# timsainb/noisereduce

Hardware: AMD Instinct MI355X
Metric: Msamples/s reduce_noise (48 kHz mono, n_fft=1024) (higher is better)
Workload: dtype f32

## Files before the change

noisereduce_amd/csrc/onepass.hpp:

```cpp
#pragma once
#include "fastpath.hpp"

namespace sg {
namespace fast {

constexpr int OP_XW = 9;
constexpr int OP_TILE_WORDS = 16 * OP_XW * 2;
constexpr int OP_MAX_NT = 16;
constexpr int OP_KP = 528;
constexpr int OP_TAB_WIN = 0, OP_TAB_WSQ = 4096, OP_TAB_INVN = 8192, OP_TAB_TW512 = 9216, OP_TAB_TW1024 = 13312,
              OP_TAB_WIN64 = 17408, OP_TAB_TW64 = 25600, OP_TAB_MCONST = 33792, OP_TAB_EXP8 = 35328, OP_TAB_BYTES = 37376;

#ifndef OP_LATE_ARGS
#define OP_LATE_ARGS 1
#endif
#ifndef OP_TRACE
#define OP_TRACE 0
#endif
#ifndef OP_ARGCHECK
#define OP_ARGCHECK 0
#endif
#ifndef OP_TILECOUNT
#define OP_TILECOUNT 0
#endif
// ... 25 lines not shown
#ifndef OP_RESTAGE
#define OP_RESTAGE 0
#endif
#ifndef OP_MAX_ITERS
#define OP_MAX_ITERS 0
#endif
#ifndef OP_LATE_START_US
#define OP_LATE_START_US 0
#endif
#ifndef OP_EXP_STALL_NS
#define OP_EXP_STALL_NS 0
#endif
#ifndef OP_INPLACE
#define OP_INPLACE 0
#endif
struct OnePassArgs {
  ApplyArgs A;
  const void* x_exact;
  int64_t stride_exact;
  int dtype_exact;
  const char* tab;
  ThreshConsts tc;
  double mag_scale, top_db;
  unsigned long long* xbits;
  unsigned* ticket;
  unsigned ticket_base;
  unsigned epoch;
  unsigned* err;
  int nf, nt;
  float prop, inv_ktot;
  unsigned long long* part2;
  unsigned* alim;
  int scan_q;
  unsigned total_tiles;
#if OP_TRACE
  unsigned* trace;
#endif
#if OP_WHO
  unsigned* who;
#endif
};

#if OP_LATE_ARGS
#define OP_XARG(type, member) (*(const __attribute__((address_space(4))) type*)(kp4 + __builtin_offsetof(OnePassArgs, member)))
#else
#define OP_XARG(type, member) (P.member)
#endif
__device__ __forceinline__ double op_exact_power(const OnePassArgs& P, int64_t row, int64_t chunk, int64_t t, int f,
                                                 int lane) {
#if OP_LATE_ARGS
  const __attribute__((address_space(4))) char* kp4 = (const __attribute__((address_space(4))) char*)__builtin_amdgcn_kernarg_segment_ptr();
  asm volatile("" : "+s"(kp4));
#endif
  const int64_t s0 = t * OP_XARG(int32_t, A.g.H) - OP_XARG(int32_t, A.g.padL);
  const int64_t v_cs = OP_XARG(int64_t, A.view.cs), v_pad = OP_XARG(int64_t, A.view.pad), v_Lp = OP_XARG(int64_t, A.view.Lp),
                v_lo = OP_XARG(int64_t, A.view.lo), v_hi = OP_XARG(int64_t, A.view.hi), x_stride = OP_XARG(int64_t, stride_exact);
  const void* const x_exact = (const void*)(uintptr_t)OP_XARG(unsigned long long, x_exact);
  const int x_dtype = OP_XARG(int, dtype_exact);
  const char* const tab = (const char*)(uintptr_t)OP_XARG(unsigned long long, tab);
  double re = 0.0, im = 0.0;
#pragma unroll 4
  for (int i = 0; i < 16; ++i) {
    const int m = lane + 64 * i;
    double xs = 0.0;
    {
      const int64_t sp = s0 + m;
      const int64_t gi = chunk * v_cs - v_pad + sp;
      if (sp >= 0 && sp < v_Lp && gi >= v_lo && gi < v_hi) xs = load_sample(x_exact, x_dtype, row * x_stride + gi);
    }
    const double xv = xs * reinterpret_cast<const double*>(tab + OP_TAB_WIN64)[m];
    const int j = (f * m) & 1023;
    cx<double> w = reinterpret_cast<const cx<double>*>(tab + OP_TAB_TW64)[j & 511];
    if (j >= 512) { w.x = -w.x; w.y = -w.y; }
    re += xv * w.x;
    im += xv * w.y;
  }
  for (int off = 32; off > 0; off >>= 1) {
    re += __shfl_xor(re, off);
    im += __shfl_xor(im, off);
  }
  return re * re + im * im;
}

#ifndef OP_ABLATE
#define OP_ABLATE 0
#endif
#ifndef OP_TRACE
#define OP_TRACE 0
#endif
#if OP_TRACE
#define OP_STAMP(i)                                                                                   \
  do {                                                                                                \
    const long long t_now_ = clock64();                                                               \
    if (lane == 0 && t_slot_) t_slot_[i] = (unsigned)(t_now_ - t_prev_);                              \
    t_prev_ = t_now_;                                                                                 \
  } while (0)
#else
#define OP_STAMP(i) do { } while (0)
#endif

#ifndef OP_LATE_P
#define OP_LATE_P 1
#endif
#ifndef OP_OCC
#define OP_OCC 3
#endif
#define OP_DONE { if (PERSIST) continue; return; }
template <int WAVES, bool PROP, bool LOSE = false, bool REDO = false, bool PERSIST = false>
__global__ __launch_bounds__(WAVES * 64, OP_OCC) void k_gate_onepass(OnePassArgs Pk) {
  static_assert(WAVES == 4, "tile = 16 frames");
  static_assert(!PERSIST || (!LOSE && !REDO), "the persistent loop is the lazy first launch only");
  extern __shared__ __attribute__((aligned(16))) char smem[];
  cf* tw512 = reinterpret_cast<cf*>(smem);
  cf* regions = tw512 + FN;
  float* swin = reinterpret_cast<float*>(regions + WAVES * WAVE_CX_H);
  float* s_t2 = swin + 1024;
  unsigned long long* s_exp = reinterpret_cast<unsigned long long*>(s_t2 + T2_FLOATS);
  double* s_t2d = reinterpret_cast<double*>(s_exp + 256);
  unsigned* s_misc = reinterpret_cast<unsigned*>(s_t2d + 514);
  unsigned char* s_ef = reinterpret_cast<unsigned char*>(s_misc + 8);
  constexpr int NF = 4 * WAVES;
  constexpr int SPAN = (NF - 1) * 256 + 1024, XPITCH = 288;
  static_assert((SPAN / 256) * XPITCH <= WAVES * WAVE_CX_H * 2, "span must fit the exchange slices");
  constexpr int NQ = SPAN / 256;
  static_assert(SPAN % 256 == 0 && WAVES * 64 == 256, "one sample per thread and row");
  constexpr int SCAN_REG = 5;

  if (REDO && Pk.alim[1] != Pk.tc.need_tag) return;
#if OP_LATE_START_US
  if (PERSIST && (blockIdx.x % 5u) == 1u) {
    const unsigned long long t0_ = wall_clock64();
    while ((long long)(wall_clock64() - t0_) < (long long)OP_LATE_START_US * 100 * (1 + (blockIdx.x % 7u))) __builtin_amdgcn_s_sleep(8);
  }
#endif
  double t2pre[3];
  unsigned alim_v = 0u;
  {
    const int tid = threadIdx.x, lane = tid & 63;
    static_assert(FN == 2 * WAVES * 64 && WAVES * 64 == 256, "one pass of the prologue loads per thread");
    const cf tw_a = reinterpret_cast<const cf*>(Pk.tab + OP_TAB_TW512)[(tid >> 4) * (tid & 15)];
    const cf tw_b = reinterpret_cast<const cf*>(Pk.tab + OP_TAB_TW512)[((tid + 256) >> 4) * (tid & 15)];
    const float4 w4 = reinterpret_cast<const float4*>(Pk.tab + OP_TAB_WIN)[tid];
    const unsigned long long e8 = reinterpret_cast<const unsigned long long*>(Pk.tab + OP_TAB_EXP8)[tid];
    t2pre[0] = Pk.tc.T2[perm_inv(tid)];
    t2pre[1] = Pk.tc.T2[perm_inv(tid + 256)];
    t2pre[2] = Pk.tc.T2[perm_inv(512)];
    if (!REDO && Pk.alim != nullptr) {
      int z = 2 + min(lane & 15, OP_ALIM_BLOCKS - 1);
      asm volatile("" : "+v"(z));
      alim_v = Pk.alim[z];
    }
    if (tid == 0) {
      s_misc[PERSIST ? 4 : 0] = Pk.ticket_base == 0xffffffffu ? blockIdx.x : atomicAdd(Pk.ticket, 1u) - Pk.ticket_base;
      s_misc[1] = 0u;
    }
    tw512[tid] = tw_a;
    tw512[tid + 256] = tw_b;
    reinterpret_cast<float4*>(swin)[tid] = w4;
    s_exp[tid] = e8;
    if constexpr (PROP) {
      for (int f = tid; f <= 512; f += WAVES * 64) {
        const int lo = max(-Pk.nf, -f), hi = min(Pk.nf, 512 - f);
        int sum = 0;
        for (int a = lo; a <= hi; ++a) sum += Pk.nf + 1 - (a < 0 ? -a : a);
        s_ef[f] = (unsigned char)sum;
      }
    }
    if constexpr (PERSIST) {
#pragma unroll
      for (int k = 0; k < 3; ++k) {
        const int i = tid + k * WAVES * 64;
        if (i > 512) break;
        s_t2[t2_pos(i)] = t2_to_f32(t2pre[k], 4.0);
        s_t2d[i] = t2pre[k];
      }
      for (int off = 1; off < 16; off <<= 1) alim_v = min(alim_v, (unsigned)__shfl_xor((int)alim_v, off));
      if (tid == 0) s_misc[2] = alim_v;
#if OP_TILECOUNT == 2
      if (tid == 0) { s_misc[3] = Pk.total_tiles; s_misc[6] = (unsigned)(uintptr_t)Pk.err; s_misc[7] = (unsigned)((uintptr_t)Pk.err >> 32); }
#endif
    }
  }
  __syncthreads();

  struct TileSrc {
    const float* sp;
    bool blk_vec;
    const float* sc_base;
    int sc_n1;
    int64_t s0b, sc_lo, sc_last, sc_lenA, sc_c0, sc_c1;
  };
  auto tile_src = [](const OnePassArgs& P, int64_t row, int64_t chunk, int jt, bool test) -> TileSrc {
    const ApplyArgs& A = P.A;
    TileSrc S;
    const int64_t tf_tile = A.h_begin - 3 + (int64_t)jt * NF;
    S.s0b = tf_tile * 256 - A.g.padL;
    const int64_t gb = chunk * A.view.cs - A.view.pad + S.s0b;
    S.sp = (const float*)A.view.x + row * A.view.stride + gb;
    S.blk_vec = A.view.dtype == 0 && tf_tile >= 0 && tf_tile + NF <= A.g.T && S.s0b >= 0 && S.s0b + SPAN <= A.view.Lp &&
                gb >= A.view.lo && gb + SPAN <= A.view.hi && (reinterpret_cast<uintptr_t>(S.sp) & 15) == 0;
    S.sc_base = nullptr;
    S.sc_n1 = 0;
    S.sc_lo = S.sc_last = S.sc_lenA = S.sc_c0 = S.sc_c1 = 0;
    if (test) {
      const int64_t g0 = chunk * A.view.cs - A.view.pad;
      const int64_t s_lo = max<int64_t>(0, A.view.lo - g0), s_hi = min<int64_t>(A.view.Lp, A.view.hi - g0);
      const int64_t sp0 = (A.h_begin - 3 - NF) * 256 - A.g.padL;
      const int64_t sp1 = (A.h_begin - 3 + (int64_t)A.n_tiles * NF) * 256 - A.g.padL + SPAN;
      const int64_t first = min(s_hi, max(s_lo, sp0));
      S.sc_lo = s_lo;
      S.sc_last = max(s_lo, min(s_hi, sp1));
      S.sc_lenA = first - s_lo;
      S.sc_c0 = (int64_t)(jt + 1) * P.scan_q;
      S.sc_c1 = min(S.sc_c0 + P.scan_q, S.sc_lenA + (s_hi - S.sc_last));
      if (A.view.dtype == 0 && S.sc_c1 > S.sc_c0 && S.sc_c1 - S.sc_c0 <= SCAN_REG * WAVES * 64 &&
          (S.sc_c1 <= S.sc_lenA || S.sc_c0 >= S.sc_lenA)) {
        S.sc_base = (const float*)A.view.x + row * A.view.stride + g0 +
                    (S.sc_c1 <= S.sc_lenA ? s_lo + S.sc_c0 : S.sc_last + (S.sc_c0 - S.sc_lenA));
        S.sc_n1 = (int)(S.sc_c1 - S.sc_c0) - 1;
      }
    }
    return S;
  };
  float q[NQ];
  float sc[SCAN_REG];
  bool pf = false;

#if OP_EXP_STALL_NS
  const unsigned long long op_exp_t0_ = wall_clock64();
#endif
  for (unsigned iter = 0; iter == 0u || PERSIST; ++iter) {
  const OnePassArgs& P = (PERSIST || OP_LATE_P) ? *late_args<OnePassArgs>() : Pk;
  int tid = threadIdx.x;
#if OP_ARGCHECK
#if OP_ARGCHECK == 2
  if (PERSIST && threadIdx.x == 1) {
    const unsigned* a_ = reinterpret_cast<const unsigned*>(&P);
    const unsigned* b_ = reinterpret_cast<const unsigned*>(&Pk);
    bool same_ = true;
    for (unsigned w_ = 0; w_ < sizeof(OnePassArgs) / 4; ++w_) same_ = same_ && a_[w_] == b_[w_];
    if (!same_) atomicOr_system(Pk.err, 0x80u);
  }
#else
  if (PERSIST && threadIdx.x == 0 && (P.total_tiles != Pk.total_tiles || P.epoch != Pk.epoch || P.xbits != Pk.xbits || P.A.view.x != Pk.A.view.x))
    atomicOr_system(Pk.err, 0x80u);
#endif
#endif
#if OP_TRACE
  long long t_prev_ = clock64();
  unsigned* t_slot_ = nullptr;
#endif
  if constexpr (PERSIST) {
    asm volatile("" : "+v"(tid));
    if (iter != 0u) {
#if !OP_NO_LOOPTOP_WAIT
      asm volatile("s_waitcnt lgkmcnt(0)" ::: "memory");
#endif
      __syncthreads();
    }
#if OP_DRAW_TOP
    if (iter != 0u) {
      if (threadIdx.x == 0) s_misc[4u + (iter & 1u)] = atomicAdd(P.ticket, 1u) - P.ticket_base;
      __syncthreads();
    }
#endif
  }
  const ApplyArgs& A = P.A;
  const Geom& G = A.g;
  const int lane = tid & 63, wave = tid >> 6;
  const int g = lane >> 4, c = lane & 15;
  const unsigned tk_slot = PERSIST ? 4u + (iter & 1u) : 0u;
  const int ntt = A.n_tiles + 2;
  const unsigned ticket = PERSIST ? (unsigned)__builtin_amdgcn_readfirstlane((int)s_misc[tk_slot]) : s_misc[0];
#if OP_TILECOUNT == 2
  if (PERSIST && threadIdx.x == 0 && P.total_tiles != s_misc[3]) {
    unsigned* e_ = (unsigned*)(((uintptr_t)s_misc[7] << 32) | (uintptr_t)s_misc[6]);
    atomicOr_system(e_, 0x40u);
    atomicMax_system(e_ + 6, P.total_tiles);
    atomicMax_system(e_ + 7, iter);
  }
  if (PERSIST && ticket >= s_misc[3]) return;
#endif
#if OP_WHO
  if (PERSIST && threadIdx.x == 0 && ticket < 4096u) P.who[ticket * 4 + 2] = (blockIdx.x + 1u) | (iter << 16);
#endif
  if (PERSIST && ticket >= P.total_tiles) return;
#if OP_TILECOUNT == 1
  if (PERSIST && threadIdx.x == 0) { atomicAdd_system(P.err + 4, 1u); atomicAdd_system(P.err + 5, ticket); }
#endif
#if OP_RESTAGE
  if (PERSIST && iter != 0u) {
    const int t_ = threadIdx.x;
    tw512[t_] = reinterpret_cast<const cf*>(P.tab + OP_TAB_TW512)[(t_ >> 4) * (t_ & 15)];
    tw512[t_ + 256] = reinterpret_cast<const cf*>(P.tab + OP_TAB_TW512)[((t_ + 256) >> 4) * (t_ & 15)];
    reinterpret_cast<float4*>(swin)[t_] = reinterpret_cast<const float4*>(P.tab + OP_TAB_WIN)[t_];
    s_exp[t_] = reinterpret_cast<const unsigned long long*>(P.tab + OP_TAB_EXP8)[t_];
#pragma unroll
    for (int k = 0; k < 3; ++k) {
      const int i = t_ + k * WAVES * 64;
      if (i > 512) break;
      const double v_ = P.tc.T2[perm_inv(i)];
      s_t2[t2_pos(i)] = t2_to_f32(v_, 4.0);
      s_t2d[i] = v_;
    }
  }
#endif
  if (PERSIST && tid == 0) {
    s_misc[1] = 0u;
#if OP_TK_LATE
    s_misc[tk_slot ^ 1u] = 0xffffffffu;
#endif
  }
#if OP_TRACE
  t_slot_ = P.trace + ((size_t)ticket * 4 + wave) * 16;
  if (lane == 0) t_slot_[14] = (blockIdx.x + 1u) | (iter << 16);
#endif
  OP_STAMP(0);
  const int64_t u = ticket / (unsigned)ntt;
  const int jt = (int)(ticket % (unsigned)ntt) - 1;
  const bool halo_tile = jt < 0 || jt >= A.n_tiles;
  const unsigned gu = (unsigned)(A.view.unit0 + u), nch = (unsigned)A.view.n_chunks;
  const int64_t row = gu / nch;
  const int64_t chunk = A.view.c0 + gu % nch;
  const bool lazy = PERSIST || P.alim != nullptr;
  const int need = (lazy && !REDO) ? 0 : need_of(P.tc, u);
  if (REDO && need == 0) return;
  if (!REDO && lazy && ticket == 0u && tid == 0) P.ticket[8] = 0u;
  const bool floor_live = need == 1;

  auto t2eff = [&](int f, double v) -> double {
    if (floor_live) {
      double fl = cell_db(P.tc.pmax[u * G.FS + f], P.mag_scale) - P.top_db;
      if (fl > P.tc.thresh[f]) v = -1.0;
    }
    if (need & 2) v = T2_NEVER;
    return v;
  };
  const int64_t tf_tile = A.h_begin - 3 + (int64_t)jt * NF;
  const int64_t tq = tf_tile + 4 * wave;
  const int64_t t = tq + g;
  const bool fvalid = t >= 0 && t < G.T;
  cf* fb = regions + wave * WAVE_CX_H + frame_base_h(g);

  bool blk_vec;
  {
    const bool test = !REDO && lazy;
    const TileSrc S = tile_src(P, row, chunk, jt, test);
    blk_vec = S.blk_vec;
    const int64_t s0b = S.s0b;
    auto fill_t2 = [&]() {
      if constexpr (!PERSIST) {
#pragma unroll
        for (int k = 0; k < 3; ++k) {
          const int i = tid + k * WAVES * 64;
          if (i > 512) break;
          const double v = t2eff(perm_inv(i), t2pre[k]);
          s_t2[t2_pos(i)] = t2_to_f32(v, 4.0);
          s_t2d[i] = v;
        }
      }
    };
    float* xs = reinterpret_cast<float*>(regions);
    unsigned mi = 0u;
    auto ab = [](float x) -> unsigned { return __float_as_uint(x) & 0x7fffffffu; };
    if (!pf) {
      if (S.blk_vec) {
#pragma unroll
        for (int k = 0; k < NQ; ++k) q[k] = S.sp[tid + k * 256];
      }
// ... 195 lines not shown
      }
      while (true) {
        const unsigned long long pending = __ballot(amb != 0 || amb512);
        if (pending == 0) break;
        const int src = __ffsll((long long)pending) - 1;
        const unsigned amb_s = (unsigned)__shfl((int)amb, src);
        const int q = amb_s ? (__ffs((int)amb_s) - 1) : 32;
        const int cs = src & 15, gs = src >> 4;
        const int f = q < 32 ? bin_of_entry(cs, q) : 512;
        const double Pe = op_exact_power(P, row, chunk, tq + gs, f, lane);
        const bool pass = Pe > s_t2d[q < 32 ? cs * 32 + q : 512];
        if (lane == src) {
          if (q < 32) {
            pred = (pred & ~(1u << q)) | ((pass ? 1u : 0u) << q);
            amb &= ~(1u << q);
          } else {
            pred512 = pass;
            amb512 = false;
          }
        }
      }
      wave_lds_sync();
#pragma unroll
      for (int i = 0; i < 16; ++i) {
        OP_PB(i).x = park[(2 * i) * 64];
        OP_PB(i).y = park[(2 * i + 1) * 64];
      }
      wave_lds_sync();
    }
    if (l0)
      pred = (pred & 0xffu) | ((pred & 0x00ffff00u) << 8) | ((pred >> 15) & 0xfe00u) | ((pred >> 23) & 0x100u);
    unsigned tr = pred;
    auto tstep = [&](int sft, unsigned msk, unsigned long long up) {
      const unsigned y = (unsigned)__shfl_xor((int)tr, sft);
      const unsigned ysh = sel_s(up, y >> sft, y << sft);
      const unsigned mk = sel_s(up, msk, ~msk);
      tr = (tr & ~mk) | (ysh & mk);
    };
    tstep(8, 0x00ff00ffu, 0xff00ff00ff00ff00ull);
    tstep(4, 0x0f0f0f0fu, 0xf0f0f0f0f0f0f0f0ull);
    tstep(2, 0x33333333u, 0xccccccccccccccccull);
    tstep(1, 0x55555555u, 0xaaaaaaaaaaaaaaaaull);
    const unsigned long long b8 = __ballot(pred512);
    {
      const int sh = 16 * g;
      const int srcl = (lane & 48) | ((2 * c) & 15);
      const unsigned wa = (unsigned)__shfl((int)tr, srcl), wb2 = (unsigned)__shfl((int)tr, srcl + 1);
      const unsigned f0 = wa & 0xffffu, f1 = wa >> 16, f2 = wb2 & 0xffffu, f3 = wb2 >> 16;
      const unsigned r1 = (((__brev(f1) >> 16) << 1) | (f1 & 1u)) & 0xffffu;
      const unsigned r3 = (((__brev(f3) >> 16) << 1) | (f3 & 1u)) & 0xffffu;
      myword = (unsigned long long)(f0 | (r1 << 16)) | ((unsigned long long)(f2 | (r3 << 16)) << 32);
      if (c == 8) myword = (b8 >> sh) & 1ull;
    }
  }

  OP_STAMP(5);
#if OP_LATE_ARGS
  typedef const __attribute__((address_space(4))) char* op_kpm_t;
  op_kpm_t kpm = (op_kpm_t)__builtin_amdgcn_kernarg_segment_ptr();
  asm volatile("" : "+s"(kpm));
#define OP_MARG(type, member) (*(const __attribute__((address_space(4))) type*)(kpm + __builtin_offsetof(OnePassArgs, member)))
  const unsigned m_ticket = (unsigned)__builtin_amdgcn_readfirstlane((int)s_misc[tk_slot]);
  const unsigned m_ntt = (unsigned)(OP_MARG(int, A.n_tiles) + 2);
  const int64_t m_u = m_ticket / m_ntt;
  const int m_jt = (int)(m_ticket % m_ntt) - 1;
#else
#define OP_MARG(type, member) (P.member)
  const unsigned m_ntt = (unsigned)ntt;
  const int64_t m_u = u;
  const int m_jt = jt;
#endif
  unsigned long long* const m_xbits = (unsigned long long*)(uintptr_t)OP_MARG(unsigned long long, xbits);
  const unsigned m_epoch = OP_MARG(unsigned, epoch);
  unsigned* const m_err = (unsigned*)(uintptr_t)OP_MARG(unsigned long long, err);
  const char* const m_tab = (const char*)(uintptr_t)OP_MARG(unsigned long long, tab);
  const float m_kscale = OP_MARG(float, A.kscale);
  const int m_nt = OP_MARG(int, nt);
  [[maybe_unused]] const float m_inv_ktot = OP_MARG(float, inv_ktot), m_prop = OP_MARG(float, prop);
  unsigned long long* xb_mine = m_xbits + ((size_t)m_u * m_ntt + (m_jt + 1)) * OP_TILE_WORDS;
  if (c < OP_XW) {
    const op_v4u gr = {(unsigned)myword, m_epoch, (unsigned)(myword >> 32), m_epoch};
    op_st16_sc1(&xb_mine[((4 * wave + g) * OP_XW + c) * 2], gr);
  }
  __syncthreads();
  if (halo_tile) {
    if constexpr (PERSIST) {
#if OP_MAX_ITERS == 1 || OP_DRAW_TOP
      if (tid == 0) s_misc[tk_slot ^ 1u] = 0xffffffffu;
#else
      if (tid == 0) s_misc[tk_slot ^ 1u] = OP_DRAW_TICKET(OP_MARG(unsigned long long, ticket)) - OP_MARG(unsigned, ticket_base);
#endif
      pf = false;
#pragma unroll
      for (int k = 0; k < NQ; ++k) q[k] = 0.f;
#pragma unroll
      for (int k = 0; k < SCAN_REG; ++k) sc[k] = 0.f;
    }
    OP_DONE;
  }
  OP_STAMP(6);

  constexpr int WP = OP_XW + 2;
  constexpr int WPB = WP * 8;
  constexpr int SLICE_B = WAVE_CX_H * 8;
  char* rbytes = reinterpret_cast<char*>(regions);
  unsigned long long* wb = reinterpret_cast<unsigned long long*>(rbytes + 4 * OP_KP * 2);
  static_assert(4 * OP_KP * 2 + 48 * WPB <= SLICE_B, "bit rows must fit behind wave 0's K rows");
  const unsigned char* wbb = reinterpret_cast<const unsigned char*>(wb);
  if (c < OP_XW) wb[(m_nt + 4 * wave + g) * WP + 1 + c] = myword;
  for (int r = tid; r < 48; r += WAVES * 64) {
    wb[r * WP] = 0ull;
    wb[r * WP + WP - 1] = 0ull;
  }
  const int q4 = lane >> 4, j16 = lane & 15;
  const long Bf = (long)reinterpret_cast<const unsigned long long*>(m_tab + OP_TAB_MCONST)[lane], At1 = (long)reinterpret_cast<const unsigned long long*>(m_tab + OP_TAB_MCONST)[64 + lane], At2 = (long)reinterpret_cast<const unsigned long long*>(m_tab + OP_TAB_MCONST)[128 + lane];
  const bool three = 2 * m_nt > 16;
  const int m1 = j16, m2 = 16 + j16;
  const int r1 = m1 < 2 * m_nt ? (m1 < m_nt ? m1 : 16 + m1) : 0;
  const int r2 = m2 < 2 * m_nt ? (m2 < m_nt ? m2 : 16 + m2) : 0;
  __syncthreads();
  typedef int op_v4i __attribute__((ext_vector_type(4)));
  const op_v4i zero4 = {0, 0, 0, 0};
  unsigned hown[9];
  {
    const unsigned char* rp = wbb + (m_nt + j16) * WPB + 7 + q4;
#pragma unroll
    for (int nb = 0; nb < 9; ++nb) {
      const int b = wave + 4 * nb;
      hown[nb] = 0u;
      if (b < 33) {
        const long a = (long)s_exp[rp[2 * b]];
        const op_v4i h = __builtin_amdgcn_mfma_i32_16x16x32_i8(a, Bf, zero4, 0, 0, 0);
        hown[nb] = (unsigned)h[0] | ((unsigned)h[1] << 8) | ((unsigned)h[2] << 16) | ((unsigned)h[3] << 24);
      }
    }
  }
  OP_STAMP(7);
  for (int i = tid; i < 2 * m_nt * OP_XW; i += WAVES * 64) {
    const int side = i >= m_nt * OP_XW;
    const int rem = i - side * m_nt * OP_XW;
    const int rr = rem / OP_XW, w = rem - rr * OP_XW;
    const unsigned long long* src = side ? xb_mine + OP_TILE_WORDS + (rr * OP_XW + w) * 2
                                         : xb_mine - OP_TILE_WORDS + ((NF - m_nt + rr) * OP_XW + w) * 2;
    op_v4u gr = op_ld16_sc1(src);
    for (int spin = 0; !(OP_ABLATE & 2) && (LOSE || gr[1] != m_epoch || gr[3] != m_epoch); ++spin) {
      if (LOSE || spin >= OP_SPIN_MAX) {
        atomicOr_system(m_err, 1u);
#if OP_WHO
        if (atomicAdd_system(m_err + 14, 1u) == 0u) { m_err[8] = m_ticket; m_err[9] = (unsigned)i; m_err[10] = gr[1]; m_err[11] = m_epoch; }
#endif
        s_misc[1] = 1u;
        break;
      }
      OP_POLL_SLEEP(spin);
      gr = op_ld16_sc1(src);
    }
    wb[(side ? m_nt + NF + rr : rr) * WP + 1 + w] = (unsigned long long)gr[0] | ((unsigned long long)gr[2] << 32);
  }
  __syncthreads();
  OP_STAMP(8);
  [[maybe_unused]] unsigned nx_raw = 0u;
  if constexpr (PERSIST) {
#if OP_MAX_ITERS == 1 || OP_DRAW_TOP
    if (tid == 0) nx_raw = 0xffffffffu + OP_MARG(unsigned, ticket_base);
#else
    if (tid == 0) nx_raw = OP_DRAW_TICKET(OP_MARG(unsigned long long, ticket));
#endif
  }
// ... 93 lines not shown
    auto merge = [&](cf& xa, cf& xb, cf w, float mk, float mn) { merge_pair(xa, xb, w, mk, mn); };
    merge(pa[0], pb[0], wlo, mval(0, ks), mval(31, ks));
    cf z0, z8;
    {
      const float y0 = (raw0.x + raw0.y) * mval(0, m_kscale);
      const float yN = (raw0.x - raw0.y) * k512;
      z0 = {0.5f * (y0 + yN), 0.5f * (y0 - yN)};
      const float m8 = mval(31, m_kscale);
      z8 = {raw8.x * m8, raw8.y * m8};
    }
#pragma unroll
    for (int sl = 1; sl < 16; ++sl) {
      const cf w = mul_tw<false>(sl < 8 ? wlo : whi, twc<32>(sl), tws<32>(sl));
      merge(pa[sl], pb[sl], w, mval(sl, ks), mval(31 - sl, ks));
    }
    v[0] = sel(z0, pa[0]);
#pragma unroll
    for (int i = 1; i < 8; ++i) v[i] = pa[i];
    v[8] = sel(z8, pa[8]);
#pragma unroll
    for (int i = 9; i < 16; ++i) v[i] = sel(pb[16 - i], pa[i]);
#pragma unroll
    for (int i = 16; i < 24; ++i) v[i] = sel(pa[i - 8], pb[31 - i]);
#pragma unroll
    for (int i = 24; i < 31; ++i) v[i] = sel(pb[39 - i], pb[31 - i]);
    v[31] = sel(pb[8], pb[0]);
  }
#endif
  wave_lds_sync();
  OP_STAMP(10);
#if OP_TK_LATE
  if constexpr (PERSIST) {
    if (tid == 0) *(volatile unsigned*)&s_misc[tk_slot ^ 1u] = nx_raw - OP_MARG(unsigned, ticket_base);
  }
#endif

  {
    int zi = 0, ci = c;
    asm volatile("" : "+v"(zi), "+v"(ci));
    fft512_inv_half(v, fb + zi, tw512 + zi, ci);
  }
  OP_STAMP(11);
  float4 n4;
  auto load_n4 = [&]() { n4 = *reinterpret_cast<const float4*>(&reinterpret_cast<const float*>(m_tab + OP_TAB_INVN)[(tid & 63) * 4]); };
  if constexpr (PERSIST) load_n4();
  auto prefetch_next = [&]() {
    const OnePassArgs& Pn = *late_args<OnePassArgs>();
#if OP_TK_LATE
    unsigned nx_v;
    while ((nx_v = *(volatile unsigned*)&s_misc[tk_slot ^ 1u]) == 0xffffffffu) __builtin_amdgcn_s_sleep(1);
    const unsigned nx = (unsigned)__builtin_amdgcn_readfirstlane((int)nx_v);
#else
    const unsigned nx = (unsigned)__builtin_amdgcn_readfirstlane((int)s_misc[tk_slot ^ 1u]);
#endif
    pf = true;
    const bool n_live = nx < Pn.total_tiles;
    const unsigned n_ntt = (unsigned)(Pn.A.n_tiles + 2);
    const unsigned n_tk = n_live ? nx : 0u;
    const unsigned n_u = n_tk / n_ntt;
    const int n_jt = (int)(n_tk % n_ntt) - 1;
    const unsigned n_gu = (unsigned)(Pn.A.view.unit0 + n_u), n_nch = (unsigned)Pn.A.view.n_chunks;
    const TileSrc N = tile_src(Pn, (int64_t)(n_gu / n_nch), Pn.A.view.c0 + n_gu % n_nch, n_jt, true);
    if (n_live && N.blk_vec) {
#pragma unroll
      for (int k = 0; k < NQ; ++k) q[k] = N.sp[tid + k * 256];
    } else {
#pragma unroll
      for (int k = 0; k < NQ; ++k) q[k] = 0.f;
    }
    if (n_live && N.sc_base != nullptr) {
#pragma unroll
      for (int k = 0; k < SCAN_REG; ++k) sc[k] = N.sc_base[min(tid + k * WAVES * 64, N.sc_n1)];
    } else {
#pragma unroll
      for (int k = 0; k < SCAN_REG; ++k) sc[k] = 0.f;
    }
  };
#ifndef OP_PF_AT
#define OP_PF_AT 2
#endif
#ifndef OP_TK_LATE
#define OP_TK_LATE 0
#endif
  if constexpr (PERSIST && OP_PF_AT == 0) prefetch_next();
  float* acc = reinterpret_cast<float*>(regions + wave * WAVE_CX_H);
  {
    const float2* wsrc2 = reinterpret_cast<const float2*>(swin + 2 * c);
#pragma unroll
    for (int j = 0; j < 4; ++j) {
#pragma unroll
      for (int rr = 0; rr < 8; ++rr) {
        const int r = 8 * j + rr;
        float2* dst = reinterpret_cast<float2*>(acc + (g + j) * HPITCH + 2 * c + 32 * rr);
        const float2 ws = wsrc2[16 * r];
        float2 nw = {v[r].x * ws.x, v[r].y * ws.y};
        if (j != 0) {
          const float2 old = *dst;
          nw.x = sel_s(OLA_KEEP, nw.x + old.x, nw.x);
          nw.y = sel_s(OLA_KEEP, nw.y + old.y, nw.y);
        }
        *dst = nw;
      }
      wave_lds_sync();
      if constexpr (PERSIST) { if (j + 1 == OP_PF_AT) prefetch_next(); }
    }
  }
  if constexpr (!PERSIST) load_n4();
  __syncthreads();
  OP_STAMP(12);
#if OP_TRACE
  if (lane == 0) t_slot_[15] = 1u;
#endif

#if OP_LATE_ARGS
  typedef const __attribute__((address_space(4))) char* op_kp_t;
  op_kp_t kp4 = (op_kp_t)__builtin_amdgcn_kernarg_segment_ptr();
  asm volatile("" : "+s"(kp4));
#define OP_KARG(type, member) (*(const __attribute__((address_space(4))) type*)(kp4 + __builtin_offsetof(OnePassArgs, member)))
#define OP_KPTR(type, member) ((type)(uintptr_t)OP_KARG(unsigned long long, member))
#else
#define OP_KARG(type, member) (P.member)
#define OP_KPTR(type, member) ((type)P.member)
#endif
  const int64_t e_gstep = OP_KARG(int64_t, A.om.g_step), e_p0 = OP_KARG(int64_t, A.om.p0), e_p1 = OP_KARG(int64_t, A.om.p1);
  void* const e_out = OP_KPTR(void*, A.om.out);
  const int64_t e_ostride = OP_KARG(int64_t, A.om.stride), e_g0 = OP_KARG(int64_t, A.om.g0), e_glo = OP_KARG(int64_t, A.om.g_lo),
                e_ghi = OP_KARG(int64_t, A.om.g_hi);
  const int e_odtype = OP_KARG(int, A.om.dtype), e_normalize = OP_KARG(int, A.normalize), e_ntiles = OP_KARG(int, A.n_tiles);
  const int64_t e_hbegin = OP_KARG(int64_t, A.h_begin), e_hend = OP_KARG(int64_t, A.h_end);
  unsigned long long* const e_part2 = OP_KPTR(unsigned long long*, part2);
  const unsigned e_epoch = OP_KARG(unsigned, epoch);
  unsigned* const e_err = OP_KPTR(unsigned*, err);
  const char* const e_tab = OP_KPTR(const char*, tab);
  const int e_padL = OP_KARG(int32_t, A.g.padL);
  const int64_t e_T = OP_KARG(int64_t, A.g.T), e_Lout = OP_KARG(int64_t, A.g.Lout);
#if OP_LATE_ARGS
  const unsigned e_ticket = (unsigned)__builtin_amdgcn_readfirstlane((int)s_misc[tk_slot]);
  const unsigned e_ntt = (unsigned)(e_ntiles + 2);
  const int64_t e_u = e_ticket / e_ntt;
  const int e_jt = (int)(e_ticket % e_ntt) - 1;
  const unsigned e_gu = (unsigned)(OP_KARG(int64_t, A.view.unit0) + e_u), e_nch = (unsigned)OP_KARG(int32_t, A.view.n_chunks);
  const int64_t e_row = e_gu / e_nch;
  const int64_t e_chunk = OP_KARG(int64_t, A.view.c0) + e_gu % e_nch;
  const int64_t e_tf = e_hbegin - 3 + (int64_t)e_jt * NF;
#else
  const int64_t e_u = u, e_row = row, e_chunk = chunk, e_tf = tf_tile;
  const int e_jt = jt;
#endif
  const float* fr = reinterpret_cast<const float*>(regions);
  const int s4 = (tid & 63) * 4;
  const float poison = s_misc[1] != 0u ? __uint_as_float(0x7fc00000u) : 0.f;
  {
    const int64_t pb0 = e_tf * 256 - e_padL;
    const int64_t gi00 = e_chunk * e_gstep + (pb0 - e_p0);
    float* dbase = (float*)e_out + (e_row * e_ostride + gi00 - e_g0);
    float* dst0 = dbase + s4;
    const bool tile_fast = e_odtype == 0 && e_normalize && e_tf >= 3 && e_tf + NF + 2 < e_T &&
                           e_tf >= e_hbegin && e_tf + NF + 2 < e_hend && pb0 >= e_p0 &&
                           pb0 + NF * 256 <= e_p1 && pb0 + NF * 256 <= e_Lout && gi00 >= e_glo &&
                           gi00 + NF * 256 <= e_ghi && (reinterpret_cast<uintptr_t>(dbase) & 15) == 0 && WAVES == 4;
    if (tile_fast) {
      constexpr int R = WAVE_CX_H * 2;
      auto ld4 = [&](int off) { return *reinterpret_cast<const float4*>(&fr[off + s4]); };
      auto fin = [&](float4 a, int jj) {
        a.x = (a.x + poison) * n4.x; a.y = (a.y + poison) * n4.y; a.z = (a.z + poison) * n4.z; a.w = (a.w + poison) * n4.w;
        *reinterpret_cast<float4*>(dst0 + jj * 256) = a;
      };
      if (wave == 3) {
#pragma unroll
        for (int it = 0; it < 4; ++it) fin(ld4(it * R + 3 * HPITCH), 3 + 4 * it);
        OP_STAMP(13);
        if constexpr (PERSIST && OP_PF_AT == 5) prefetch_next();
        OP_DONE;
      }
      {
        const float4 a4 = ld4((WAVES - 1) * R + (wave + 4) * HPITCH);
        unsigned long long* dst = e_part2 + (((size_t)e_u * e_ntiles + e_jt) * 3 + wave) * 256 + s4;
        const op_v4u ga = {__float_as_uint(a4.x + poison), e_epoch, __float_as_uint(a4.y + poison), e_epoch};
        const op_v4u gb = {__float_as_uint(a4.z + poison), e_epoch, __float_as_uint(a4.w + poison), e_epoch};
        op_st16_sc1(dst, ga);
        op_st16_sc1(dst + 2, gb);
      }
#pragma unroll
      for (int it = 1; it < 4; ++it) {
        float4 a4 = ld4((it - 1) * R + (wave + 4) * HPITCH);
        const float4 f4 = ld4(it * R + wave * HPITCH);
        a4.x += f4.x; a4.y += f4.y; a4.z += f4.z; a4.w += f4.w;
        fin(a4, wave + 4 * it);
      }
      {
        float4 a4 = ld4(wave * HPITCH);
        const unsigned long long* src = e_part2 + (((size_t)e_u * e_ntiles + e_jt - 1) * 3 + wave) * 256 + s4;
        op_v4u ga, gb;
        for (int spin = 0;; ++spin) {
          asm volatile("global_load_dwordx4 %0, %2, off sc1\n\tglobal_load_dwordx4 %1, %2, off offset:16 sc1\n\ts_waitcnt vmcnt(0)"
                       : "=&v"(ga), "=&v"(gb) : "v"(src) : "memory");
          const unsigned e = e_epoch;
          if ((OP_ABLATE & 16) || (!LOSE && ga[1] == e && ga[3] == e && gb[1] == e && gb[3] == e)) break;
          if (LOSE || spin >= OP_SPIN_MAX) {
            atomicOr_system(e_err, 2u);
#if OP_WHO
            if (atomicAdd_system(e_err + 15, 1u) == 0u) { e_err[12] = e_ticket; e_err[13] = ga[1]; }
#endif
            ga[0] = ga[2] = gb[0] = gb[2] = 0x7fc00000u;
            break;
          }
          OP_POLL_SLEEP(spin);
        }
        a4.x = __uint_as_float(ga[0]) + a4.x;
        a4.y = __uint_as_float(ga[2]) + a4.y;
        a4.z = __uint_as_float(gb[0]) + a4.z;
        a4.w = __uint_as_float(gb[2]) + a4.w;
        fin(a4, wave);
      }
      OP_STAMP(13);
      if constexpr (PERSIST && OP_PF_AT == 5) prefetch_next();
      OP_DONE;
    }
  }
  for (int it = 0; it < 5; ++it) {
    const int jj = wave < 3 ? (it == 0 ? NF + wave : (it == 4 ? wave : wave + 4 * it)) : (it < 4 ? 3 + 4 * it : -1);
    if (jj < 0) break;
    const int64_t h = e_tf + jj;
    if (h >= e_hend || h < e_hbegin) continue;
    float4 a4 = make_float4(0.f, 0.f, 0.f, 0.f);
    bool all_valid = true;
#pragma unroll
    for (int q = 0; q < 4; ++q) {
      const int64_t ti = e_tf + jj - q;
      if (ti < 0 || ti >= e_T) all_valid = false;
    }
    {
      const int wh = jj >> 2, lh = jj & 3;
      if (wh >= 1 && wh - 1 < WAVES && lh <= 2) {
        a4 = *reinterpret_cast<const float4*>(&fr[(wh - 1) * WAVE_CX_H * 2 + (lh + 4) * HPITCH + s4]);
      }
      if (wh < WAVES) {
        const float4 f4 = *reinterpret_cast<const float4*>(&fr[wh * WAVE_CX_H * 2 + lh * HPITCH + s4]);
        a4.x += f4.x; a4.y += f4.y; a4.z += f4.z; a4.w += f4.w;
      }
    }
    if (jj >= NF) {
      const int k = jj - NF;
      unsigned long long* dst = e_part2 + (((size_t)e_u * e_ntiles + e_jt) * 3 + k) * 256 + s4;
      const op_v4u ga = {__float_as_uint(a4.x + poison), e_epoch, __float_as_uint(a4.y + poison), e_epoch};
      const op_v4u gb = {__float_as_uint(a4.z + poison), e_epoch, __float_as_uint(a4.w + poison), e_epoch};
      op_st16_sc1(dst, ga);
      op_st16_sc1(dst + 2, gb);
      continue;
    }
    if (jj < 3) {
      const unsigned long long* src = e_part2 + (((size_t)e_u * e_ntiles + e_jt - 1) * 3 + jj) * 256 + s4;
      op_v4u ga, gb;
      for (int spin = 0;; ++spin) {
        asm volatile("global_load_dwordx4 %0, %2, off sc1\n\tglobal_load_dwordx4 %1, %2, off offset:16 sc1\n\ts_waitcnt vmcnt(0)"
                     : "=&v"(ga), "=&v"(gb) : "v"(src) : "memory");
        const unsigned e = e_epoch;
        if ((OP_ABLATE & 16) || (!LOSE && ga[1] == e && ga[3] == e && gb[1] == e && gb[3] == e)) break;
        if (LOSE || spin >= OP_SPIN_MAX) {
          atomicOr_system(e_err, 2u);
          ga[0] = ga[2] = gb[0] = gb[2] = 0x7fc00000u;
          break;
        }
        OP_POLL_SLEEP(spin);
      }
      a4.x = __uint_as_float(ga[0]) + a4.x;
      a4.y = __uint_as_float(ga[2]) + a4.y;
      a4.z = __uint_as_float(gb[0]) + a4.z;
      a4.w = __uint_as_float(gb[2]) + a4.w;
    }
    a4.x += poison; a4.y += poison; a4.z += poison; a4.w += poison;
    if (!e_normalize) {
    } else if (all_valid) {
      a4.x *= n4.x; a4.y *= n4.y; a4.z *= n4.z; a4.w *= n4.w;
    } else {
      float4 nrm = make_float4(0.f, 0.f, 0.f, 0.f);
#pragma unroll
      for (int q = 0; q < 4; ++q) {
        const int64_t ti = h - q;
        if (ti >= 0 && ti < e_T) {
          const float4 w4 = *reinterpret_cast<const float4*>(&reinterpret_cast<const float*>(e_tab + OP_TAB_WSQ)[256 * q + s4]);
          nrm.x += w4.x; nrm.y += w4.y; nrm.z += w4.z; nrm.w += w4.w;
        }
      }
      a4.x /= (nrm.x > 1e-10f ? nrm.x : 1.f);
      a4.y /= (nrm.y > 1e-10f ? nrm.y : 1.f);
      a4.z /= (nrm.z > 1e-10f ? nrm.z : 1.f);
      a4.w /= (nrm.w > 1e-10f ? nrm.w : 1.f);
    }
    {
      const int64_t pb = h * 256 - e_padL;
      const int64_t gi0 = e_chunk * e_gstep + (pb - e_p0);
      if (e_odtype == 0 && pb >= e_p0 && pb + 256 <= e_p1 && pb + 256 <= e_Lout && gi0 >= e_glo &&
          gi0 + 256 <= e_ghi) {
        float* dst = (float*)e_out + (e_row * e_ostride + gi0 - e_g0 + s4);
        if ((reinterpret_cast<uintptr_t>(dst) & 15) == 0) {
          *reinterpret_cast<float4*>(dst) = a4;
          continue;
        }
      }
    }
    const float vals[4] = {a4.x, a4.y, a4.z, a4.w};
#pragma unroll
    for (int e = 0; e < 4; ++e) {
      const int64_t p = h * 256 + s4 + e - e_padL;
      if (p < e_p0 || p >= e_p1) continue;
      const int64_t gi = e_chunk * e_gstep + (p - e_p0);
      if (gi < e_glo || gi >= e_ghi) continue;
      store_sample(e_out, e_odtype, e_row * e_ostride + gi - e_g0, p < e_Lout ? vals[e] : 0.f);
    }
  }
  if constexpr (PERSIST && OP_PF_AT == 5) prefetch_next();
  }
}

}
}
```

Measured before the change: 101,300.

## Defer seam overlap-add to next persistent tile to hide cross-tile wait

```diff
diff --git a/noisereduce_amd/csrc/onepass.hpp b/noisereduce_amd/csrc/onepass.hpp
--- a/noisereduce_amd/csrc/onepass.hpp
+++ b/noisereduce_amd/csrc/onepass.hpp
@@ -131,6 +131,12 @@
   return re * re + im * im;
 }
 
+__device__ __forceinline__ unsigned op_nan_bits() {
+  unsigned v = 0x7fc00000u;
+  asm volatile("" : "+v"(v));
+  return v;
+}
+
 #ifndef OP_ABLATE
 #define OP_ABLATE 0
 #endif
@@ -155,6 +161,10 @@
 #define OP_OCC 3
 #endif
 #define OP_DONE { if (PERSIST) continue; return; }
+#ifndef OP_DEFER_SEAM
+#define OP_DEFER_SEAM 1
+#endif
+constexpr unsigned OP_SEAM_NONE = 0xffffffffu;
 template <int WAVES, bool PROP, bool LOSE = false, bool REDO = false, bool PERSIST = false>
 __global__ __launch_bounds__(WAVES * 64, OP_OCC) void k_gate_onepass(OnePassArgs Pk) {
   static_assert(WAVES == 4, "tile = 16 frames");
@@ -202,6 +212,7 @@
     if (tid == 0) {
       s_misc[PERSIST ? 4 : 0] = Pk.ticket_base == 0xffffffffu ? blockIdx.x : atomicAdd(Pk.ticket, 1u) - Pk.ticket_base;
       s_misc[1] = 0u;
+      if (PERSIST) s_misc[0] = OP_SEAM_NONE;
     }
     tw512[tid] = tw_a;
     tw512[tid + 256] = tw_b;
@@ -274,6 +285,80 @@
   float q[NQ];
   float sc[SCAN_REG];
   bool pf = false;
+  constexpr bool DEFER = PERSIST && OP_DEFER_SEAM;
+  auto seam_where = [](unsigned pend, const unsigned long long*& src, float*& dst) {
+    typedef const __attribute__((address_space(4))) char* kq_t;
+    kq_t kq = (kq_t)__builtin_amdgcn_kernarg_segment_ptr();
+    asm volatile("" : "+s"(kq));
+#define OP_QARG(type, member) (*(const __attribute__((address_space(4))) type*)(kq + __builtin_offsetof(OnePassArgs, member)))
+    const unsigned tk = pend & 0x7fffffffu;
+    const unsigned ntl = (unsigned)OP_QARG(int, A.n_tiles), nttq = ntl + 2u;
+    const unsigned uq = tk / nttq;
+    const int jq = (int)(tk % nttq) - 1;
+    const unsigned guq = (unsigned)(OP_QARG(int64_t, A.view.unit0) + uq), nchq = (unsigned)OP_QARG(int32_t, A.view.n_chunks);
+    const int64_t rowq = guq / nchq, chunkq = OP_QARG(int64_t, A.view.c0) + guq % nchq;
+    const int64_t tfq = OP_QARG(int64_t, A.h_begin) - 3 + (int64_t)jq * NF;
+    const int64_t pb0 = tfq * 256 - OP_QARG(int32_t, A.g.padL);
+    const int64_t gi00 = chunkq * OP_QARG(int64_t, A.om.g_step) + (pb0 - OP_QARG(int64_t, A.om.p0));
+    auto uni = [](const void* p_) -> char* {
+      const unsigned long long v_ = (unsigned long long)(uintptr_t)p_;
+      return (char*)(uintptr_t)(((unsigned long long)(unsigned)__builtin_amdgcn_readfirstlane((int)(v_ >> 32)) << 32) |
+                                (unsigned)__builtin_amdgcn_readfirstlane((int)v_));
+    };
+    dst = (float*)uni((float*)(uintptr_t)OP_QARG(unsigned long long, A.om.out) +
+                      (rowq * OP_QARG(int64_t, A.om.stride) + gi00 - OP_QARG(int64_t, A.om.g0)));
+    src = (const unsigned long long*)uni((const unsigned long long*)(uintptr_t)OP_QARG(unsigned long long, part2) +
+                                         ((size_t)uq * ntl + jq - 1) * 3 * 256);
+  };
+  auto seam_off = [](int wv, int s4_) -> int { return wv * 256 + s4_; };
+  auto seam_finish = [&](unsigned pend, int wv, int s4_, unsigned long long g0_, unsigned long long g1_, unsigned long long g2_,
+                        unsigned long long g3_, float* dst, float4 ld, float4 nrm) {
+    op_v4u ga = {(unsigned)g0_, (unsigned)(g0_ >> 32), (unsigned)g1_, (unsigned)(g1_ >> 32)};
+    op_v4u gb = {(unsigned)g2_, (unsigned)(g2_ >> 32), (unsigned)g3_, (unsigned)(g3_ >> 32)};
+    typedef const __attribute__((address_space(4))) char* kq_t;
+    kq_t kq = (kq_t)__builtin_amdgcn_kernarg_segment_ptr();
+    asm volatile("" : "+s"(kq));
+    const unsigned e = OP_QARG(unsigned, epoch);
+    if (!(ga[1] == e && ga[3] == e && gb[1] == e && gb[3] == e)) {
+      const unsigned long long* src;
+      float* d2_;
+      seam_where(pend, src, d2_);
+      src += seam_off(wv, s4_);
+      for (int spin = 0;; ++spin) {
+        asm volatile("global_load_dwordx4 %0, %2, off sc1\n\tglobal_load_dwordx4 %1, %2, off offset:16 sc1\n\ts_waitcnt vmcnt(0)"
+                     : "=&v"(ga), "=&v"(gb) : "v"(src) : "memory");
+        if (ga[1] == e && ga[3] == e && gb[1] == e && gb[3] == e) break;
+        if (spin >= OP_SPIN_MAX) {
+          atomicOr_system((unsigned*)(uintptr_t)OP_QARG(unsigned long long, err), 2u);
+          ga[0] = ga[2] = gb[0] = gb[2] = op_nan_bits();
+          break;
+        }
+        OP_POLL_SLEEP(spin);
+      }
+    }
+    const float psn = __uint_as_float((pend >> 31) * 0x7fc00000u);
+    float4 a;
+    a.x = __uint_as_float(ga[0]) + ld.x;
+    a.y = __uint_as_float(ga[2]) + ld.y;
+    a.z = __uint_as_float(gb[0]) + ld.z;
+    a.w = __uint_as_float(gb[2]) + ld.w;
+    a.x = (a.x + psn) * nrm.x; a.y = (a.y + psn) * nrm.y; a.z = (a.z + psn) * nrm.z; a.w = (a.w + psn) * nrm.w;
+    *reinterpret_cast<float4*>(dst + seam_off(wv, s4_)) = a;
+  };
+  auto seam_close = [&](unsigned pend, int tid_) {
+    const int wv = tid_ >> 6, s4_ = (tid_ & 63) * 4;
+    if (pend == OP_SEAM_NONE || wv >= 3) return;
+    typedef const __attribute__((address_space(4))) char* kq_t;
+    kq_t kq = (kq_t)__builtin_amdgcn_kernarg_segment_ptr();
+    asm volatile("" : "+s"(kq));
+    const float4 nrm = *reinterpret_cast<const float4*>(
+        &reinterpret_cast<const float*>((const char*)(uintptr_t)OP_QARG(unsigned long long, tab) + OP_TAB_INVN)[s4_]);
+    const unsigned long long* src;
+    float* dst;
+    seam_where(pend, src, dst);
+    const float4 ld = *reinterpret_cast<const float4*>(dst + seam_off(wv, s4_));
+    seam_finish(pend, wv, s4_, 0ull, 0ull, 0ull, 0ull, dst, ld, nrm);
+  };
 
 #if OP_EXP_STALL_NS
   const unsigned long long op_exp_t0_ = wall_clock64();
@@ -333,7 +418,10 @@
 #if OP_WHO
   if (PERSIST && threadIdx.x == 0 && ticket < 4096u) P.who[ticket * 4 + 2] = (blockIdx.x + 1u) | (iter << 16);
 #endif
-  if (PERSIST && ticket >= P.total_tiles) return;
+  if (PERSIST && ticket >= P.total_tiles) {
+    if constexpr (DEFER) seam_close((unsigned)__builtin_amdgcn_readfirstlane((int)s_misc[0]), tid);
+    return;
+  }
 #if OP_TILECOUNT == 1
   if (PERSIST && threadIdx.x == 0) { atomicAdd_system(P.err + 4, 1u); atomicAdd_system(P.err + 5, ticket); }
 #endif
@@ -695,8 +783,16 @@
     const op_v4u gr = {(unsigned)myword, m_epoch, (unsigned)(myword >> 32), m_epoch};
     op_st16_sc1(&xb_mine[((4 * wave + g) * OP_XW + c) * 2], gr);
   }
+  [[maybe_unused]] unsigned pend_halo = OP_SEAM_NONE;
+  if constexpr (DEFER) {
+    if (halo_tile) pend_halo = (unsigned)__builtin_amdgcn_readfirstlane((int)s_misc[0]);
+  }
   __syncthreads();
   if (halo_tile) {
+    if constexpr (DEFER) {
+      seam_close(pend_halo, tid);
+      if (tid == 0) s_misc[0] = OP_SEAM_NONE;
+    }
     if constexpr (PERSIST) {
 #if OP_MAX_ITERS == 1 || OP_DRAW_TOP
       if (tid == 0) s_misc[tk_slot ^ 1u] = 0xffffffffu;
@@ -956,6 +1052,28 @@
 #ifndef OP_TK_LATE
 #define OP_TK_LATE 0
 #endif
+#ifndef OP_SEAM_AT
+#define OP_SEAM_AT 4
+#endif
+  [[maybe_unused]] unsigned sm_pend = OP_SEAM_NONE;
+  [[maybe_unused]] unsigned long long sm_g0 = 0ull, sm_g1 = 0ull, sm_g2 = 0ull, sm_g3 = 0ull;
+  [[maybe_unused]] float* sm_dst = nullptr;
+  [[maybe_unused]] float4 sm_lead = make_float4(0.f, 0.f, 0.f, 0.f);
+  auto seam_issue = [&]() {
+    sm_pend = (unsigned)__builtin_amdgcn_readfirstlane((int)s_misc[0]);
+    if (sm_pend != OP_SEAM_NONE && wave < 3) {
+      const unsigned long long* sm_src;
+      seam_where(sm_pend, sm_src, sm_dst);
+      sm_src += seam_off(wave, (tid & 63) * 4);
+      sm_g0 = __hip_atomic_load((const __attribute__((address_space(1))) unsigned long long*)(sm_src), __ATOMIC_RELAXED, __HIP_MEMORY_SCOPE_AGENT);
+      sm_g1 = __hip_atomic_load((const __attribute__((address_space(1))) unsigned long long*)(sm_src + 1), __ATOMIC_RELAXED, __HIP_MEMORY_SCOPE_AGENT);
+      sm_g2 = __hip_atomic_load((const __attribute__((address_space(1))) unsigned long long*)(sm_src + 2), __ATOMIC_RELAXED, __HIP_MEMORY_SCOPE_AGENT);
+      sm_g3 = __hip_atomic_load((const __attribute__((address_space(1))) unsigned long long*)(sm_src + 3), __ATOMIC_RELAXED, __HIP_MEMORY_SCOPE_AGENT);
+      typedef float op_v4f __attribute__((ext_vector_type(4)));
+      const op_v4f l4 = *(const __attribute__((address_space(1))) op_v4f*)(sm_dst + seam_off(wave, (tid & 63) * 4));
+      sm_lead = make_float4(l4[0], l4[1], l4[2], l4[3]);
+    }
+  };
   if constexpr (PERSIST && OP_PF_AT == 0) prefetch_next();
   float* acc = reinterpret_cast<float*>(regions + wave * WAVE_CX_H);
   {
@@ -977,6 +1095,7 @@
       }
       wave_lds_sync();
       if constexpr (PERSIST) { if (j + 1 == OP_PF_AT) prefetch_next(); }
+      if constexpr (DEFER) { if (j + 1 == OP_SEAM_AT) seam_issue(); }
     }
   }
   if constexpr (!PERSIST) load_n4();
@@ -1020,10 +1139,13 @@
 #else
   const int64_t e_u = u, e_row = row, e_chunk = chunk, e_tf = tf_tile;
   const int e_jt = jt;
+  [[maybe_unused]] const unsigned e_ticket = ticket;
 #endif
   const float* fr = reinterpret_cast<const float*>(regions);
   const int s4 = (tid & 63) * 4;
-  const float poison = s_misc[1] != 0u ? __uint_as_float(0x7fc00000u) : 0.f;
+  unsigned poison_u = __builtin_amdgcn_readfirstlane((int)s_misc[1]) != 0 ? 0x7fc00000u : 0u;
+  asm volatile("" : "+s"(poison_u));
+  const float poison = __uint_as_float(poison_u);
   {
     const int64_t pb0 = e_tf * 256 - e_padL;
     const int64_t gi00 = e_chunk * e_gstep + (pb0 - e_p0);
@@ -1062,7 +1184,11 @@
         a4.x += f4.x; a4.y += f4.y; a4.z += f4.z; a4.w += f4.w;
         fin(a4, wave + 4 * it);
       }
-      {
+      if constexpr (DEFER) {
+        if (sm_pend != OP_SEAM_NONE) seam_finish(sm_pend, wave, s4, sm_g0, sm_g1, sm_g2, sm_g3, sm_dst, sm_lead, n4);
+        *reinterpret_cast<float4*>(dst0 + wave * 256) = ld4(wave * HPITCH);
+        if (tid == 0) s_misc[0] = e_ticket | (s_misc[1] != 0u ? 0x80000000u : 0u);
+      } else {
         float4 a4 = ld4(wave * HPITCH);
         const unsigned long long* src = e_part2 + (((size_t)e_u * e_ntiles + e_jt - 1) * 3 + wave) * 256 + s4;
         op_v4u ga, gb;
@@ -1076,7 +1202,7 @@
 #if OP_WHO
             if (atomicAdd_system(e_err + 15, 1u) == 0u) { e_err[12] = e_ticket; e_err[13] = ga[1]; }
 #endif
-            ga[0] = ga[2] = gb[0] = gb[2] = 0x7fc00000u;
+            ga[0] = ga[2] = gb[0] = gb[2] = op_nan_bits();
             break;
           }
           OP_POLL_SLEEP(spin);
@@ -1091,6 +1217,10 @@
       if constexpr (PERSIST && OP_PF_AT == 5) prefetch_next();
       OP_DONE;
     }
+  }
+  if constexpr (DEFER) {
+    if (sm_pend != OP_SEAM_NONE && wave < 3) seam_finish(sm_pend, wave, s4, sm_g0, sm_g1, sm_g2, sm_g3, sm_dst, sm_lead, n4);
+    if (tid == 0) s_misc[0] = OP_SEAM_NONE;
   }
   for (int it = 0; it < 5; ++it) {
     const int jj = wave < 3 ? (it == 0 ? NF + wave : (it == 4 ? wave : wave + 4 * it)) : (it < 4 ? 3 + 4 * it : -1);
@@ -1133,7 +1263,7 @@
         if ((OP_ABLATE & 16) || (!LOSE && ga[1] == e && ga[3] == e && gb[1] == e && gb[3] == e)) break;
         if (LOSE || spin >= OP_SPIN_MAX) {
           atomicOr_system(e_err, 2u);
-          ga[0] = ga[2] = gb[0] = gb[2] = 0x7fc00000u;
+          ga[0] = ga[2] = gb[0] = gb[2] = op_nan_bits();
           break;
         }
         OP_POLL_SLEEP(spin);
```

After: 103,200 (median of 6 runs). +1.9%, better.
